# victorkich/ManyTor

Hardware: AMD Instinct MI355X
Metric: env-steps/sec (whole node), 1M parallel 4-DoF arms, random actions (higher is better)
Workload: dtype f32

## Files before the change

### manytor_amd/csrc/engine.hip

```cpp
#include <hip/hip_runtime.h>

#include <algorithm>
#include <cmath>
#include <cstdio>
#include <cstdlib>
#include <cstring>
#include <mutex>
#include <new>
#include <iterator>
#include <string>
#include <utility>
#include <vector>

#include "engine_internal.h"
#include "kernels.h"

using namespace mt;

namespace {
thread_local std::string g_last_error;
}

namespace mt {
int fail(mt_handle h, int code, const std::string& msg) {
// ... 148 lines not shown
  if (env_int("MT_RESET_SPLIT", &v)) {
    h->reset_split = v != 0;
    seen("MT_RESET_SPLIT");
  }
  h->graph_mode = -1;
  h->graph_max = P.graph_max;
  if (env_int("MT_GRAPH", &v)) {
    h->graph_mode = v != 0 ? 1 : 0;
    seen("MT_GRAPH");
  }
  h->flat_from = P.flat_from;
  if (env_int("MT_FLAT_FROM", &v)) {
    h->flat_from = std::max<long long>(0, v);
    seen("MT_FLAT_FROM");
  }
  h->blocks_per_cu_override = -1;
  if (env_int("MT_BLOCKS_PER_CU", &v)) {
    const int c = (int)std::max<long long>(0, std::min<long long>(8, v));
    h->blocks_per_cu_override = (c == 1 || c == 2) ? 3 : c;
    seen("MT_BLOCKS_PER_CU");
  }
  h->trig_steps = h->static_kind != 0;
  if (env_int("MT_TRIG_TABLE", &v)) {
    h->trig_steps = v != 0 && h->static_kind != 0;
    seen("MT_TRIG_TABLE");
  }

  h->chains = (n >= P.chains_min && n <= P.chains_max) ? 2 : 1;
  h->chains_forced = false;
  if (env_int("MT_CHAINS", &v)) {
    h->chains = (int)std::max<long long>(1, std::min<long long>(mt_engine::kMaxChains, v));
    h->chains_forced = true;
    seen("MT_CHAINS");
  }
  if (n < 2 * 256) h->chains = 1;
  h->lazy_chains = true;
  if (env_int("MT_LAZY_CHAINS", &v)) {
    h->lazy_chains = v != 0;
    seen("MT_LAZY_CHAINS");
  }

  h->multi_k = (n <= P.multi_step_max) ? P.multi_step_k : 1;
  if (env_int("MT_ROLLOUT_K", &v)) {
    h->multi_k = (int)std::max<long long>(1, std::min<long long>(64, v));
    seen("MT_ROLLOUT_K");
  }
  h->defer_reset = true;
  if (env_int("MT_DEFER_RESET", &v)) {
    h->defer_reset = v != 0;
    seen("MT_DEFER_RESET");
  }
  h->defer_reset_chained = P.fold_reset_into_chains;
  if (env_int("MT_DEFER_RESET_CHAINS", &v)) {
    h->defer_reset_chained = v != 0;
    seen("MT_DEFER_RESET_CHAINS");
  }
  h->gather_throttle = true;
  if (env_int("MT_GATHER_THROTTLE", &v)) {
    h->gather_throttle = v != 0;
    seen("MT_GATHER_THROTTLE");
  }
  h->snap_in_rollout = true;
  if (env_int("MT_ROLLOUT_SNAP", &v)) {
    h->snap_in_rollout = v != 0;
    seen("MT_ROLLOUT_SNAP");
  }
  h->rollout_early = true;
  if (env_int("MT_ROLLOUT_EARLY", &v)) {
    h->rollout_early = v != 0;
    seen("MT_ROLLOUT_EARLY");
  }

  h->tape_prefetch = false;
  if (env_int("MT_TAPE_PREFETCH", &v)) {
    h->tape_prefetch = v != 0;
    seen("MT_TAPE_PREFETCH");
  }
  h->tape_nt_loads = false;
  if (env_int("MT_TAPE_NT", &v)) {
    h->tape_nt_loads = v != 0;
    seen("MT_TAPE_NT");
  }

  if (h->custom_frames) h->lds_table = false;
  auto schedule_for = [&](int64_t envs, int64_t split4_max, int64_t split2_max, int64_t prefetch_other_max) {
    mt_engine::Schedule s;
    s.step_lanes = envs <= split4_max ? 4 : (envs <= split2_max ? 2 : 1);
    s.prefetch = h->static_kind == 1 || envs <= prefetch_other_max;
    s.rollout_lanes = envs <= P.fused_split4_max ? 4 : (envs <= P.fused_split2_max ? 2 : 1);
    if (forced_lanes) s.step_lanes = s.rollout_lanes = forced_lanes;
    if (forced_prefetch >= 0) s.prefetch = forced_prefetch != 0;
    if (h->custom_frames) s = mt_engine::Schedule{};
    return s;
  };
  h->sched[mt_engine::kBatch] = schedule_for(n, P.step_split4_max, P.step_split2_max, P.prefetch_other_max);
  h->sched[mt_engine::kChain] =
      h->chains > 1 ? schedule_for(chain_span(h, h->chains), P.chain_split4_max, P.chain_split2_max, P.chain_prefetch_other_max)
                    : h->sched[mt_engine::kBatch];
}

#define MT_DISPATCH_D(D_, FN, ...)   \
  switch (D_) {                      \
    case 2: FN<2>(__VA_ARGS__); break; \
    case 3: FN<3>(__VA_ARGS__); break; \
    case 4: FN<4>(__VA_ARGS__); break; \
    case 5: FN<5>(__VA_ARGS__); break; \
    case 6: FN<6>(__VA_ARGS__); break; \
    case 7: FN<7>(__VA_ARGS__); break; \
    case 8: FN<8>(__VA_ARGS__); break; \
    default: break;                  \
  }

struct StepVariant {
  int trig = 0;
  bool lds = false;
  int lanes = 1;
  int pf = 0;
  bool tt = false;
  bool flat = false;
  bool fresh = false;
  bool codes = false;
};
constexpr unsigned variant_key(const StepVariant& v) {
  return (unsigned)v.trig | (unsigned)v.lds << 3 | (unsigned)v.lanes << 4 | (unsigned)(v.pf != 0) << 7 | (unsigned)v.tt << 8 |
         (unsigned)v.flat << 9 | (unsigned)v.fresh << 10 | (unsigned)v.codes << 11;
}

#pragma clang diagnostic push
#pragma clang diagnostic ignored "-Wc++20-designator"
constexpr StepVariant kRuntimeVariants[] = {
    {.trig = 0}, {.trig = 1}, {.trig = 2}, {.trig = 3}, {.trig = 4}, {.trig = 5},
    {.lds = true},
    {.lanes = 2}, {.lanes = 4},
    {.pf = kPrefetch}, {.pf = kPrefetch, .flat = true},
};
constexpr StepVariant kFramesVariants[] = {{.trig = 0}, {.trig = 1}};
constexpr StepVariant kStaticVariants[] = {
    {.trig = 0}, {.trig = 1}, {.trig = 2}, {.trig = 3}, {.trig = 4}, {.trig = 5},
    {.lanes = 2}, {.lanes = 4},
    {.lanes = 2, .tt = true}, {.lanes = 4, .tt = true},
    {.pf = kPrefetch}, {.pf = kPrefetch, .flat = true},
    {.pf = 0, .tt = true}, {.pf = kPrefetch, .tt = true}, {.pf = kPrefetch, .tt = true, .flat = true},
    {.pf = kPrefetch, .tt = true, .codes = true}, {.pf = kPrefetch, .tt = true, .flat = true, .codes = true},
    {.pf = 0, .tt = true, .fresh = true}, {.pf = kPrefetch, .tt = true, .fresh = true},
    {.pf = kPrefetch, .tt = true, .flat = true, .fresh = true},
};
#pragma clang diagnostic pop

enum class TableKind { kRuntime = 0, kRef4 = 1, kDh7 = 2, kFrames = 3 };
struct StepPlan {
  TableKind table = TableKind::kRuntime;
  int D = 0;
  bool sample = false;
  StepVariant v;
  int blocks_per_cu = 0;
  size_t lds_bytes = 0;
  dim3 grid;
  bool exists = true;
};

StepPlan plan_step(const mt_engine* h, mt_engine::Scope scope, int64_t n, bool sample, bool codes, bool fresh = false) {
  const mt_engine::Schedule& s = h->sched[scope == mt_engine::kChain ? mt_engine::kChain : mt_engine::kBatch];
  const bool whole_rows = scope != mt_engine::kOneEnv;
  StepPlan p;
  p.table = h->custom_frames ? TableKind::kFrames : (TableKind)h->static_kind;
  p.D = h->D;
  p.sample = sample;
  p.grid = grid_for(n);
  StepVariant& v = p.v;
  if (fresh) {
    const size_t stage = (size_t)2 * h->K * kBlock * sizeof(float), fixed = kTrigEntries * sizeof(SinCos) + 512;
    p.exists = h->trig == 0 && h->trig_steps && s.step_lanes == 1 && !h->lds_table && !h->trace &&
               stage + fixed <= 65536;
    if (!p.exists) return p;
    p.sample = true;
    v.tt = v.fresh = true;
    v.pf = s.prefetch ? kPrefetch : 0;
    v.flat = v.pf && n >= h->flat_from;
    p.blocks_per_cu = v.pf ? step_blocks_per_cu(h, n) : 0;
    p.lds_bytes = std::max(stage, lds_pad_for_blocks(p.blocks_per_cu, fixed));
    return p;
  }
  if (p.table == TableKind::kFrames) {
    v.trig = h->trig == 1 ? 1 : 0;
    return p;
  }
  if (h->lds_table) {
    v.lds = true;
    return p;
  }
  if (h->trig != 0) {
    v.trig = h->trig;
    return p;
  }
  v.tt = sample && h->trig_steps && whole_rows;
  if (s.step_lanes > 1) {
    v.lanes = s.step_lanes;
    const int64_t per_block = kBlock / v.lanes;
    p.grid = dim3((unsigned)((n + per_block - 1) / per_block));
    return p;
  }
  v.pf = s.prefetch ? kPrefetch : 0;
  v.flat = v.pf && n >= h->flat_from;
  v.codes = v.pf && v.tt && codes;
  if (v.pf && v.tt) {
    p.blocks_per_cu = step_blocks_per_cu(h, n);
    p.lds_bytes = lds_pad_for_blocks(p.blocks_per_cu, kTrigEntries * sizeof(SinCos));
  }
  return p;
}

template <class Tbl, bool SAMPLE, const auto& ROWS, size_t I>
void launch_variant(const StepPlan& p, hipStream_t stream, const StepArgs& args) {
  constexpr StepVariant V = ROWS[I];
  if constexpr (V.lanes > 1)
    hipLaunchKernelGGL((step_split_kernel<Tbl, SAMPLE, V.lanes, V.tt>), p.grid, dim3(kBlock), p.lds_bytes, stream, args);
  else
    hipLaunchKernelGGL((step_kernel<Tbl, SAMPLE, V.trig, V.lds, V.pf, V.tt, V.flat, V.fresh, V.codes>), p.grid, dim3(kBlock),
                       p.lds_bytes, stream, args);
}
template <class Tbl, const auto& ROWS, size_t I>
bool launch_row(const StepPlan& p, hipStream_t stream, const StepArgs& args) {
  if (variant_key(p.v) != variant_key(ROWS[I])) return false;
  if (p.sample)
    launch_variant<Tbl, true, ROWS, I>(p, stream, args);
  else if constexpr (!ROWS[I].tt)
    launch_variant<Tbl, false, ROWS, I>(p, stream, args);
  else
    return false;
  return true;
}
template <class Tbl, const auto& ROWS, size_t... I>
bool launch_rows(const StepPlan& p, hipStream_t stream, const StepArgs& args, std::index_sequence<I...>) {
  return (launch_row<Tbl, ROWS, I>(p, stream, args) || ...);
}
template <class Tbl, const auto& ROWS>
bool launch_table(const StepPlan& p, hipStream_t stream, const StepArgs& args) {
  return launch_rows<Tbl, ROWS>(p, stream, args, std::make_index_sequence<std::size(ROWS)>{});
}
template <int D>
void launch_plan_d(const StepPlan& p, hipStream_t stream, const StepArgs& args, bool* launched) {
  *launched = p.table == TableKind::kFrames ? launch_table<RtTableF<D>, kFramesVariants>(p, stream, args)
                                            : launch_table<RtTable<D>, kRuntimeVariants>(p, stream, args);
}

void launch_plan(const StepPlan& p, hipStream_t stream, const StepArgs& args) {
  bool launched = false;
  if (p.table == TableKind::kRef4)
    launched = launch_table<Ref4Table, kStaticVariants>(p, stream, args);
  else if (p.table == TableKind::kDh7)
    launched = launch_table<Dh7Table, kStaticVariants>(p, stream, args);
  else
    MT_DISPATCH_D(p.D, launch_plan_d, p, stream, args, &launched);
  if (!launched) {
    std::fprintf(stderr, "manytor: no step kernel for table %d, D %d, sample %d, variant key 0x%x\n", (int)p.table, p.D,
                 (int)p.sample, variant_key(p.v));
    std::abort();
  }
}

template <int D>
void launch_trace_d(mt_handle h, const StepArgs& args, float* trace, bool sample) {
  if (sample)
    hipLaunchKernelGGL((trace_kernel<D, true>), grid_for(args.n), dim3(kBlock), 0, h->stream, args, trace);
  else
    hipLaunchKernelGGL((trace_kernel<D, false>), grid_for(args.n), dim3(kBlock), 0, h->stream, args, trace);
}

void launch_step(mt_handle h, mt_engine::Scope scope, const StepArgs& args, float* trace, bool sample) {
  if (trace) MT_DISPATCH_D(h->D, launch_trace_d, h, args, trace, sample);
  const StepPlan p = plan_step(h, scope, args.n, sample, h->codes_valid);
  launch_plan(p, h->stream, args);
  h->codes_valid = p.v.codes;
}

void launch_step(mt_handle h, bool sample) { launch_step(h, mt_engine::kBatch, h->args, h->trace, sample); }

bool launch_step_fresh(mt_handle h, mt_engine::Scope scope, const StepArgs& args) {
  const StepPlan p = plan_step(h, scope, args.n, true, false, true);
  if (!p.exists) return false;
  launch_plan(p, h->stream, args);
  h->codes_valid = p.v.codes;
  return true;
}

StepArgs args_for_range(mt_handle h, const StepArgs& base, int64_t off, int64_t cnt);
int check_launch(mt_handle h, const char* what);
int ensure_chains(mt_handle h, int chains) {
  if (!h->ev_fork) MT_HIP(h, hipEventCreateWithFlags(&h->ev_fork, event_flags(false)));
  for (int c = 1; c < chains; ++c) {
    if (!h->chain_streams[c]) MT_HIP(h, hipStreamCreateWithFlags(&h->chain_streams[c], hipStreamNonBlocking));
    if (!h->ev_join[c]) MT_HIP(h, hipEventCreateWithFlags(&h->ev_join[c], event_flags(false)));
  }
  return MT_OK;
}

void launch_chain(mt_handle h, const StepArgs& a0, uint32_t major0, int T, int chains, int c, bool sample = true) {
  const int64_t span = chain_span(h, chains), off = (int64_t)c * span;
  if (off >= h->n) return;
  StepArgs as = args_for_range(h, a0, off, std::min(span, h->n - off));
  for (int s = 0; s < T; ++s) {
    as.major = major0 + (uint32_t)s;
    launch_step(h, mt_engine::kChain, as, nullptr, sample);
  }
}

bool launch_chain_fresh(mt_handle h, const StepArgs& a0, uint32_t major, int chains, int c) {
  const int64_t span = chain_span(h, chains), off = (int64_t)c * span;
  if (off >= h->n) return true;
  StepArgs as = args_for_range(h, a0, off, std::min(span, h->n - off));
  as.major = major;
  return launch_step_fresh(h, mt_engine::kChain, as);
}

hipStream_t chain_stream(mt_handle h, int c) { return c == 0 ? h->stream : h->chain_streams[c]; }

int fork_chains(mt_handle h, int chains) {
  if (h->forked) return MT_OK;
  int rc = ensure_chains(h, chains);
  if (rc) return rc;
  const int64_t span = chain_span(h, chains);
  MT_HIP(h, hipEventRecord(h->ev_fork, h->stream));
  for (int c = 1; c < chains; ++c)
    if ((int64_t)c * span < h->n) MT_HIP(h, hipStreamWaitEvent(h->chain_streams[c], h->ev_fork, 0));
  h->forked = true;
  return MT_OK;
}

int settle_chains(mt_handle h) { return (h->lazy_chains && h->stream == h->own_stream) ? MT_OK : join_chains(h); }

// ... 432 lines not shown
    }
    if (h->ev_join[c]) (void)hipEventDestroy(h->ev_join[c]);
    if (h->ev1c[c]) (void)hipEventDestroy(h->ev1c[c]);
  }
  if (h->ev_fork) (void)hipEventDestroy(h->ev_fork);
  if (h->graph_step0) (void)hipFree(h->graph_step0);
  if (h->staging) (void)hipFree(h->staging);
  if (h->pinned) (void)hipHostFree(h->pinned);
  if (h->arena) (void)hipFree(h->arena);
  if (h->ev0) (void)hipEventDestroy(h->ev0);
  if (h->ev1) (void)hipEventDestroy(h->ev1);
  for (hipEvent_t e : h->lap_events) (void)hipEventDestroy(e);
  if (h->own_stream) (void)hipStreamDestroy(h->own_stream);
  delete h;
  return MT_OK;
}

static StepPlan batch_plan(const mt_engine* h) { return plan_step(h, mt_engine::kBatch, h->n, true, false); }
static StepPlan chain_plan(const mt_engine* h) { return plan_step(h, mt_engine::kChain, chain_span(h, h->chains), true, false); }
static std::string table_name(const mt_engine* h) {
  const char* tbl = h->static_kind == 1 ? "Ref4Table" : (h->static_kind == 2 ? "Dh7Table" : nullptr);
  return tbl ? tbl : (h->custom_frames ? "RtTableF<" : "RtTable<") + std::to_string(h->D) + ">";
}
static int multi_step_lanes(const mt_engine* h) {
  return h->sched[(h->chains > 1 && h->chains_forced) ? mt_engine::kChain : mt_engine::kBatch].rollout_lanes;
}

const char* mt_step_kernel_name(mt_handle h) {
  if (!h) return "";
  const std::string table = table_name(h);
  const StepVariant v = batch_plan(h).v;
  if (v.lanes > 1)
    h->kernel_name = "step_split_kernel<" + table + ", L=" + std::to_string(v.lanes) + (v.tt ? ", tt=1>" : ">");
  else
    h->kernel_name = "step_kernel<" + table + ", trig=" + std::to_string(h->trig) + ", lds=" + (v.lds ? "true" : "false") +
                     ", pf=" + std::to_string(v.pf) + (v.tt ? ", tt=1" : "") + (v.flat ? ", flat=1>" : ">");
  const bool multi_one_chain = h->multi_k > 1 && fusable(h) && !h->chains_forced;
  if (h->chains > 1 && !multi_one_chain) {
    const StepPlan c = chain_plan(h);
    h->kernel_name += " [mt_rollout: " + std::to_string(h->chains) + " chains of " + std::to_string(chain_span(h, h->chains)) +
                      " envs, " + (c.v.lanes > 1 ? "L=" + std::to_string(c.v.lanes)
                                                 : "pf=" + std::to_string(c.v.pf) + (c.v.flat ? ", flat=1" : "")) +
                      (c.blocks_per_cu > 0 ? ", " + std::to_string(c.blocks_per_cu) + " blocks/CU" : std::string()) + "]";
  }
  if (h->multi_k > 1 && fusable(h)) {
    const int sp = multi_step_lanes(h);
    h->kernel_name += " [mt_rollout: " + std::to_string(h->multi_k) + " steps per launch, " +
                      (sp > 1 ? "rollout_split_kernel L=" + std::to_string(sp) : std::string("rollout_kernel")) + "]";
  }
  return h->kernel_name.c_str();
}

const char* mt_describe_dispatch(mt_handle h) {
  if (!h) return "";
  const DispatchPolicy& P = kPolicy;
  auto num = [](long long v) { return std::to_string(v); };
  auto b = [](bool v) { return std::string(v ? "true" : "false"); };
  const int64_t span = chain_span(h, h->chains);
  const std::string table = table_name(h);
  const StepPlan sb = batch_plan(h), sc = chain_plan(h);
  const bool multi = h->multi_k > 1 && fusable(h);
  const bool graph = h->graph_mode > 0 || (h->graph_mode < 0 && h->n <= h->graph_max);
  std::string caps = "[";
  for (const BlockCap& c : P.block_caps) caps += std::string(caps.size() > 1 ? "," : "") + "[" + num(c.from) + "," + num(c.below) + "," + num(c.blocks) + "]";
  caps += "]";
  std::string& d = h->describe;
  d = "{\"n_envs\":" + num(h->n) + ",\"ld\":" + num(h->ld) + ",\"dof\":" + num(h->D) + ",\"targets\":" + num(h->K) +
      ",\"table\":\"" + table + "\",\"trig\":" + num(h->trig) + ",\"lds_table\":" + b(h->lds_table) + ",\"custom_frames\":" + b(h->custom_frames) +
      ",\"step\":{\"lanes_per_env\":" + num(sb.v.lanes) + ",\"prefetch\":" + b(sb.v.pf != 0) +
      ",\"trig_table\":" + b(sb.v.tt) + ",\"flat\":" + b(sb.v.flat) + "}" +
      ",\"chains\":{\"count\":" + num(h->chains) + ",\"span\":" + num(h->chains > 1 ? span : h->n) + ",\"lazy\":" + b(h->lazy_chains) +
      ",\"lanes_per_env\":" + num(sc.v.lanes) + ",\"prefetch\":" + b(sc.v.pf != 0) + ",\"flat\":" + b(sc.v.flat) +
      ",\"blocks_per_cu\":" + num(h->chains > 1 ? sc.blocks_per_cu : 0) + "}" +
      ",\"rollout\":{\"form\":\"" + (multi ? "multi_step" : (h->chains > 1 ? "chained_steps" : (graph ? "graph_replay" : "launch_per_step"))) +
      "\",\"steps_per_launch\":" + num(multi ? h->multi_k : 1) + ",\"graph\":" + b(!multi && graph) +
      ",\"lanes_per_env\":" + num(multi ? multi_step_lanes(h) : (h->chains > 1 ? sc : sb).v.lanes) +
      ",\"chains\":" + num(multi && !h->chains_forced ? 1 : h->chains) +
      ",\"absorbs_reset\":" + b(h->defer_reset && (multi || chained_rollout_absorbs_reset(h))) + ",\"writes_snapshot\":" + b(h->snap_in_rollout && (multi || (h->chains > 1 && !graph && !h->trace))) + "}" +
      ",\"fused\":{\"usable\":" + b(fusable(h)) + ",\"lanes_per_env\":" + num(h->sched[mt_engine::kBatch].rollout_lanes) + "}" +
      ",\"tape\":{\"usable\":" + b(fusable(h)) + ",\"lanes_per_env\":1,\"chains\":1,\"prefetch\":" + b(tape_prefetches(h)) +
      ",\"nt_loads\":" + b(h->tape_nt_loads) + "}" +
      ",\"shoot\":{\"usable\":" + b(fusable(h)) + ",\"envs_per_block\":" + num(kShootEnvs) + ",\"waves_per_block\":" + num(kShootWaves) + "}" +
      ",\"reset\":{\"lanes_per_env\":" + num(h->reset_split ? 4 : 1) + "}" +
      ",\"overrides\":\"" + h->overrides + "\"" +
      ",\"policy\":{\"step_split4_max\":" + num(P.step_split4_max) + ",\"step_split2_max\":" + num(P.step_split2_max) +
      ",\"prefetch_other_max\":" + num(P.prefetch_other_max) + ",\"fused_split4_max\":" + num(P.fused_split4_max) +
      ",\"fused_split2_max\":" + num(P.fused_split2_max) + ",\"reset_split_max\":" + num(P.reset_split_max) +
      ",\"graph_max\":" + num(P.graph_max) + ",\"chains_min\":" + num(P.chains_min) + ",\"chains_max\":" + num(P.chains_max) +
      ",\"chain_split4_max\":" + num(P.chain_split4_max) + ",\"chain_split2_max\":" + num(P.chain_split2_max) +
      ",\"chain_prefetch_other_max\":" + num(P.chain_prefetch_other_max) + ",\"flat_from\":" + num(P.flat_from) +
      ",\"block_caps\":" + caps + ",\"multi_step_max\":" + num(P.multi_step_max) + ",\"multi_step_k\":" + num(P.multi_step_k) +
      ",\"max_recurrence_rotations\":" + num(P.max_recurrence_rotations) + ",\"ld_pad_above\":" + num(P.ld_pad_above) +
      ",\"ld_pad_floats\":" + num(P.ld_pad_floats) + "}" +
      ",\"arena_bytes\":" + num((long long)h->arena_bytes) + "}";
  return d.c_str();
}

int mt_set_stream(mt_handle h, void* hip_stream) {
  MT_REQUIRE(nullptr, h != nullptr, "handle is NULL");
  MT_ENTER(h);
  MT_HIP(h, hipStreamSynchronize(h->stream));
  h->stream = (hipStream_t)hip_stream;
  return MT_OK;
}

int mt_use_own_stream(mt_handle h) {
  MT_REQUIRE(nullptr, h != nullptr, "handle is NULL");
  MT_ENTER(h);
  MT_HIP(h, hipStreamSynchronize(h->stream));
  h->stream = h->own_stream;
  return MT_OK;
}

int mt_sync(mt_handle h) {
  MT_REQUIRE(nullptr, h != nullptr, "handle is NULL");
  MT_ENTER(h);
  MT_HIP(h, hipStreamSynchronize(h->stream));
  if (h->gather_pending) {
    MT_HIP(h, hipStreamSynchronize(h->side_stream));
    MT_HIP(h, hipEventElapsedTime(&h->last_gather_ms, h->ev_g0, h->ev_g1));
    h->gather_pending = false;
    h->snap_free_known[0] = h->snap_free_known[1] = true;
  }
  return MT_OK;
}

int mt_reset(mt_handle h, const float* points, int layout, int is_device) {
  MT_REQUIRE(nullptr, h != nullptr, "handle is NULL");
  MT_REQUIRE(h, points != nullptr, "points is NULL (use mt_reset_random for device-drawn targets)");
  MT_REQUIRE(h, layout == MT_ENV_MAJOR || layout == MT_SOA, "bad layout");
  if (!is_device && layout == MT_ENV_MAJOR) {
    const int64_t bad = first_unusable(points, h->n * 3 * h->K, kMaxFiniteBits);
    if (bad >= 0) return fail(h, MT_ERR_INVALID_ARG, "mt_reset: points element " + std::to_string(bad) + " is NaN or infinite");
  }
  if (!is_device && layout == MT_SOA)
    for (int r = 0; r < 3 * h->K; ++r) {
      const int64_t bad = first_unusable(points + (int64_t)r * h->ld, h->n, kMaxFiniteBits);
      if (bad >= 0)
        return fail(h, MT_ERR_INVALID_ARG, "mt_reset: points row " + std::to_string(r) + " element " + std::to_string(bad) + " is NaN or infinite");
    }
  MT_ENTER(h);
  const int rows = 3 * h->K;
  if (layout == MT_SOA) {
    const size_t bytes = (size_t)rows * h->ld * 4;
    MT_HIP(h, hipMemcpyAsync(h->args.points, points, bytes, is_device ? hipMemcpyDeviceToDevice : hipMemcpyHostToDevice,
                             h->stream));
  } else {
    const size_t bytes = (size_t)rows * h->n * 4;
    const float* src = points;
    if (!is_device) {
      int rc = ensure_staging(h, bytes);
      if (rc) return rc;
      MT_HIP(h, hipMemcpyAsync(h->staging, points, bytes, hipMemcpyHostToDevice, h->stream));
      src = (const float*)h->staging;
    }
    hipLaunchKernelGGL((env_major_to_soa<float>), grid_for(h->n), dim3(kBlock), 0, h->stream, src, rows, h->n,
                       h->args.points, h->ld);
    int rc = check_launch(h, "env_major_to_soa");
    if (rc) return rc;
  }
  {
    int rcg = order_behind_inplace_gather(h, h->stream);
    if (rcg) return rcg;
  }
  h->args.major = 0;
  h->args.episode0 = 0;
// ... 1259 lines not shown
```

### manytor_amd/csrc/engine_internal.h

```cpp
#pragma once
#include <hip/hip_runtime.h>

#include <cstdlib>
#include <string>
#include <vector>

#include "step_args.h"

struct mt_comm;

struct mt_engine {
  static constexpr int kMaxChains = 4;
  mt_config cfg{};
  int64_t n = 0, ld = 0;
  int D = 0, K = 0;
  hipStream_t own_stream = nullptr;
  hipStream_t stream = nullptr;
  hipEvent_t ev0 = nullptr, ev1 = nullptr;
  hipEvent_t ev1c[kMaxChains] = {nullptr, nullptr, nullptr, nullptr};
  int timer_ends = 0;
  bool timer_with_gather = false;
  struct LapRec {
    uint32_t begin, n_begin, end0, n_end;
  };
  std::vector<hipEvent_t> lap_events;
  size_t lap_events_used = 0;
  std::vector<LapRec> lap_recs;
  bool lap_open = false;
  void* arena = nullptr;
  size_t arena_bytes = 0;
  void* staging = nullptr;
  size_t staging_bytes = 0;
  void* pinned = nullptr;
  size_t pinned_bytes = 0;
  mt::StepArgs args{};
  float* trace = nullptr;
  unsigned long long* spare_bits = nullptr;
  bool is_reset = false;
  int trig = 0;
  bool lds_table = false;
  bool custom_frames = false;
  struct Schedule {
    int step_lanes = 1;
    bool prefetch = false;
    int rollout_lanes = 1;
  };
  enum Scope { kBatch = 0, kChain = 1, kOneEnv = 2 };
  Schedule sched[2];
  int blocks_per_cu_override = -1;
  int64_t flat_from = 393216;
  bool goals_exposed = false;
  bool codes_valid = false;
  bool points_exposed = false;
  bool trig_steps = false;
  int static_kind = 0;
  mt_comm* comm = nullptr;
  hipStream_t side_stream = nullptr;
  hipEvent_t ev_snap = nullptr, ev_g0 = nullptr, ev_g1 = nullptr;
  float* snap = nullptr;
  hipEvent_t ev_gdone[2] = {nullptr, nullptr};
  bool snap_free_known[2] = {true, true};
  int snap_next = 0;
  bool gather_throttle = true;
  float* snap_row(int p) const { return snap + (size_t)p * (size_t)n; }
  void* reduce_scratch = nullptr;
  size_t reduce_scratch_bytes = 0;
  bool reset_split = false;
  struct RolloutGraph {
    int T;
    int chains;
    mt::StepArgs args;
    hipGraphExec_t exec[kMaxChains];
  };
  std::vector<RolloutGraph> graphs;
  std::vector<int> graph_seen;
  uint32_t* graph_step0 = nullptr;
  int graph_mode = -1;
  int64_t graph_max = 131072;
  int chains = 1;
  bool chains_forced = false;
  int multi_k = 1;
  bool rollout_early = true;
  bool defer_reset_chained = false;
  bool defer_reset = true;
  bool reset_pending = false;
  uint64_t pend_seed = 0;
  uint32_t pend_episode = 0;
  bool snap_in_rollout = true;
  bool snap_valid = false;
  bool tape_prefetch = false;
  bool tape_nt_loads = false;
  std::string overrides;
  std::string describe;
  hipStream_t chain_streams[kMaxChains] = {nullptr, nullptr, nullptr, nullptr};
  hipEvent_t ev_fork = nullptr, ev_join[kMaxChains] = {nullptr, nullptr, nullptr, nullptr};
  bool forked = false;
  bool lazy_chains = true;
  bool gather_pending = false;
  bool gather_inplace = false;
  float last_gather_ms = 0.f;
  std::string err;
  std::string kernel_name;
};

namespace mt {

inline unsigned event_flags(bool timing) {
  static const bool fenced = [] {
    const char* e = std::getenv("MT_EVENT_FENCE");
    return e && *e && std::atoi(e) != 0;
  }();
  return (timing ? 0u : (unsigned)hipEventDisableTiming) | (fenced ? 0u : (unsigned)hipEventDisableSystemFence);
}

int fail(mt_handle h, int code, const std::string& msg);

class DeviceGuard {
 public:
  explicit DeviceGuard(int device) {
    if (hipGetDevice(&prev_) != hipSuccess) prev_ = -1;
    err_ = (prev_ == device) ? hipSuccess : hipSetDevice(device);
    changed_ = (err_ == hipSuccess && prev_ != device);
  }
  ~DeviceGuard() {
    if (changed_ && prev_ >= 0) (void)hipSetDevice(prev_);
  }
  hipError_t error() const { return err_; }

 private:
  int prev_ = -1;
  hipError_t err_ = hipSuccess;
  bool changed_ = false;
};

inline dim3 grid_for(int64_t n) { return dim3((unsigned)((n + kBlock - 1) / kBlock)); }

inline bool snapshot_trusted(mt_engine* h) {
  if (h->stream != h->own_stream) return false;
  hipStreamCaptureStatus st = hipStreamCaptureStatusNone;
  if (hipStreamIsCapturing(h->stream, &st) != hipSuccess) {
    (void)hipGetLastError();
    return false;
  }
  return st == hipStreamCaptureStatusNone;
}

int join_chains(mt_handle h);
int flush_pending_reset(mt_handle h);

}

#define MT_HIP(h, call)                                                                            \
  do {                                                                                             \
    hipError_t e__ = (call);                                                                       \
    if (e__ != hipSuccess)                                                                         \
      return mt::fail(h, MT_ERR_HIP, std::string(#call) + ": " + hipGetErrorString(e__));          \
  } while (0)

#define MT_REQUIRE(h, cond, msg)                              \
  do {                                                        \
    if (!(cond)) return mt::fail(h, MT_ERR_INVALID_ARG, msg); \
  } while (0)

#define MT_ON_DEVICE(h, device)                                                                          \
  mt::DeviceGuard mt_guard__(device);                                                                    \
  if (mt_guard__.error() != hipSuccess)                                                                  \
  return mt::fail(h, MT_ERR_HIP, std::string("hipSetDevice: ") + hipGetErrorString(mt_guard__.error()))

#define MT_ENTER(h)                              \
  MT_ON_DEVICE(h, (h)->cfg.device);              \
  do {                                           \
    (h)->snap_valid = false;                     \
    if ((h)->forked) {                           \
      int rcj__ = mt::join_chains(h);            \
// ... 20 lines not shown
```

### manytor_amd/csrc/kernels.h

```cpp
#pragma once
#include <hip/hip_runtime.h>
#include <stdint.h>

#include "mt_math.h"
#include "philox.h"
#include "step_args.h"

namespace mt {

#ifndef MT_NT_STORES
#define MT_NT_STORES 1
#endif
template <typename T>
using global_ptr = __attribute__((address_space(1))) T*;

__device__ __forceinline__ global_ptr<char> uniform_row(const void* row) {
  const uint64_t v = reinterpret_cast<uint64_t>(row);
  const uint32_t lo = __builtin_amdgcn_readfirstlane((uint32_t)v);
  const uint32_t hi = __builtin_amdgcn_readfirstlane((uint32_t)(v >> 32));
  return (global_ptr<char>)(((uint64_t)hi << 32) | lo);
}
#ifndef MT_PLAIN_LANE_OFFSET
#define MT_PLAIN_LANE_OFFSET 0
#endif
template <bool RENEW>
struct LaneOffset {
  uint32_t v;
};
template <bool RENEW>
__device__ __forceinline__ uint32_t lane_offset(LaneOffset<RENEW>& o) {
#if !MT_PLAIN_LANE_OFFSET
  if (RENEW) asm volatile("" : "+v"(o.v));
#endif
  return o.v;
}
#ifndef MT_BUFFER_ROWS
#define MT_BUFFER_ROWS 0
#endif
#if MT_BUFFER_ROWS
constexpr int kRsrcWord3 = 0x00020000;
constexpr int kAuxNt = 2;
__device__ __forceinline__ __amdgpu_buffer_rsrc_t row_rsrc(const void* row) {
  return __builtin_amdgcn_make_buffer_rsrc((void*)uniform_row(row), 0, -1, kRsrcWord3);
}
template <typename T, bool R>
__device__ __forceinline__ T ldr(const T* row, LaneOffset<R>& o) {
  static_assert(sizeof(T) == 4 || sizeof(T) == 1, "rows hold 32-bit words or bytes");
  if constexpr (sizeof(T) == 4)
    return __builtin_bit_cast(T, __builtin_amdgcn_raw_buffer_load_b32(row_rsrc(row), (int)o.v, 0, 0));
  else
    return __builtin_bit_cast(T, __builtin_amdgcn_raw_buffer_load_b8(row_rsrc(row), (int)o.v, 0, 0));
}
template <typename T, bool R>
__device__ __forceinline__ void str(T* row, LaneOffset<R>& o, T v) {
  static_assert(sizeof(T) == 4 || sizeof(T) == 1, "rows hold 32-bit words or bytes");
  if constexpr (sizeof(T) == 4)
    __builtin_amdgcn_raw_buffer_store_b32(__builtin_bit_cast(uint32_t, v), row_rsrc(row), (int)o.v, 0, 0);
  else
    __builtin_amdgcn_raw_buffer_store_b8(__builtin_bit_cast(uint8_t, v), row_rsrc(row), (int)o.v, 0, 0);
}
template <typename T, bool R>
__device__ __forceinline__ void str_stream(T* row, LaneOffset<R>& o, T v) {
  static_assert(sizeof(T) == 4 || sizeof(T) == 1, "rows hold 32-bit words or bytes");
  constexpr int aux = MT_NT_STORES ? kAuxNt : 0;
  if constexpr (sizeof(T) == 4)
    __builtin_amdgcn_raw_buffer_store_b32(__builtin_bit_cast(uint32_t, v), row_rsrc(row), (int)o.v, 0, aux);
  else
    __builtin_amdgcn_raw_buffer_store_b8(__builtin_bit_cast(uint8_t, v), row_rsrc(row), (int)o.v, 0, aux);
}
#else
template <typename T, bool R>
__device__ __forceinline__ T ldr(const T* row, LaneOffset<R>& o) {
  return *(global_ptr<const T>)(uniform_row(row) + lane_offset(o));
}
template <typename T, bool R>
__device__ __forceinline__ void str(T* row, LaneOffset<R>& o, T v) {
  *(global_ptr<T>)(uniform_row(row) + lane_offset(o)) = v;
}
template <typename T, bool R>
__device__ __forceinline__ void str_stream(T* row, LaneOffset<R>& o, T v) {
  global_ptr<T> p = (global_ptr<T>)(uniform_row(row) + lane_offset(o));
#if MT_NT_STORES
  __builtin_nontemporal_store(v, p);
#else
  *p = v;
// ... 506 lines not shown
      for (int j = 1; j < JN; ++j) {
        const float pose = __builtin_fmaf(fk, st[j], gq[j]);
        if (TRIG == 2)
          sincos_deg_hw(pose, sF[j], cF[j]);
        else
          sincos_deg(pose, sF[j], cF[j]);
      }
      chain_z<Tbl>(sF, cF, t, zo, ze);
      zmin = fminf(zmin, fminf(zo, ze));
    }
  }
  return zmin;
}

template <class Tbl, bool TABLE>
__device__ __forceinline__ bool wide_route(const float (&g)[Tbl::D], const float (&act)[Tbl::D], bool prev_whole) {
  float reach = 0.f;
  if (!prev_whole) {
#pragma unroll
    for (int j = 0; j < Tbl::D; ++j) reach = fmaxf(reach, __builtin_fabsf(g[j]));
  }
  if (!TABLE) {
#pragma unroll
    for (int j = 0; j < Tbl::D; ++j) reach = fmaxf(reach, __builtin_fabsf(act[j]));
  }
  return wide_angle(reach);
}

template <class Tbl, bool CACHED>
__device__ __forceinline__ float route_kinematics_wide(const Tbl& t, int S, const float (&g)[Tbl::D],
                                                       const float (&act)[Tbl::D], float (&el)[3], float (&e)[3],
                                                       PoseCache<Tbl::D>* cache) {
  constexpr int D = Tbl::D;
  constexpr int JN = ZJoints<Tbl>::value;
  float s[D], c[D];
#pragma unroll
  for (int j = 0; j < D; ++j) {
    s[j] = 0.f;
    c[j] = 1.f;
  }
  float zmin = 0.f;
  const double inv = 1.0 / (double)(S - 1);
  for (int k = 0; k < S - 1; ++k) {
    const double frac = (double)k * inv;
#pragma unroll
    for (int j = 1; j < JN; ++j) {
      float gj = g[j], aj = act[j];
      asm volatile("" : "+v"(gj), "+v"(aj));
      sincos_deg_route(gj, aj, frac, t.off(j), s[j], c[j]);
    }
    float zo, ze;
    chain_z<Tbl>(s, c, t, zo, ze);
    zmin = (k == 0) ? fminf(zo, ze) : fminf(zmin, fminf(zo, ze));
  }
  float p[D][3];
#pragma unroll
  for (int j = 0; j < D; ++j) sincos_deg_off(act[j], t.off(j), s[j], c[j]);
  chain_all<Tbl>(s, c, t, p);
  pick_frames<Tbl>(t, p, el, e);
  if (CACHED) {
#pragma unroll
    for (int j = 1; j < JN; ++j) {
      cache->s[j] = s[j];
      cache->c[j] = c[j];
    }
    cache->zmin = fminf(el[2], e[2]);
  }
  zmin = fminf(zmin, fminf(el[2], e[2]));
  return zmin;
}

template <class Tbl, int TRIG, bool CACHED = false, bool TABLE = false>
__device__ __forceinline__ float route_kinematics(const Tbl& t, int S, float inv_sm1, const float (&g)[Tbl::D],
                                                  const float (&act)[Tbl::D], float (&el)[3], float (&e)[3],
                                                  PoseCache<Tbl::D>* cache = nullptr, bool cache_valid = false,
                                                  const SinCos* trig = nullptr, bool prev_whole = false) {
  if constexpr (TRIG <= 2) {
    if (__builtin_expect(__any(wide_route<Tbl, TABLE>(g, act, prev_whole)), 0))
      return route_kinematics_wide<Tbl, CACHED>(t, S, g, act, el, e, cache);
  }
  return route_kinematics_narrow<Tbl, TRIG, CACHED, TABLE>(t, S, inv_sm1, g, act, el, e, cache, cache_valid, trig, prev_whole);
}

__device__ __forceinline__ void record_finished(const StepArgs& a, uint32_t i, uint32_t episode, float ret) {
  LaneOffset<true> o4{i * 4u};
  str(a.last_return, o4, ret);
  if (a.ring_slots)
    a.ring[(int64_t)((episode - a.episode0) % a.ring_slots) * a.ld + i] = ret;
}

#ifdef MT_STAMPS
#define MT_STAMP(a, i, slot)                                                                 \
  do {                                                                                       \
    __builtin_amdgcn_sched_barrier(0);                                                       \
    unsigned long long t__;                                                                  \
    asm volatile("s_memtime %0\n\ts_waitcnt lgkmcnt(0)" : "=s"(t__)::"memory");              \
    __builtin_amdgcn_sched_barrier(0);                                                       \
    if ((a).stamps && (threadIdx.x & 63) == 0) (a).stamps[(size_t)((i) >> 6) * 8 + (slot)] = t__; \
  } while (0)
#else
#define MT_STAMP(a, i, slot) \
  do {                       \
  } while (0)
#endif

__device__ __forceinline__ bool unusable_angle(float v) { return (__float_as_uint(v) & 0x7FFFFFFFu) > 0x47000000u; }

template <class Tbl, int TRIG>
constexpr int step_min_waves() { return (TRIG == 0 && Tbl::D >= 6 && Tbl::D <= 7) ? 8 : 1; }

constexpr int kPrefetch = 8;

__device__ __forceinline__ void draw_targets_wave(uint64_t seed, uint64_t env0, uint32_t episode, bool need, int K, float radius,
                                                  float* col0, uint8_t* slots);

template <class Tbl, bool SAMPLE, int TRIG, bool LDS, int PF = 0, bool TT = false, bool FLAT = false, bool FRESH = false,
          bool CODES = false>
__global__ __launch_bounds__(kBlock, (PF ? 1 : step_min_waves<Tbl, TRIG>())) void step_kernel(const StepArgs a) {
  constexpr int D = Tbl::D;
  static_assert(!TT || (SAMPLE && TRIG == 0 && !LDS && ActionTrigTable<Tbl>::value), "the table serves sampled actions of a static table");
  static_assert(!FRESH || TT, "the reset prologue exists for the sampled-action kernels of the static tables");
  static_assert(!CODES || (PF && TT && !FRESH), "codes are read by the prefetch kernels of the static tables");
  extern __shared__ float fresh_stage[];
  __shared__ uint8_t fresh_slots[FRESH ? kBlock / 64 : 1][64];
  __shared__ DhConst sh;
  __shared__ __attribute__((aligned(16))) SinCos trig_lds[TT ? kTrigEntries : 1];
  float4 trig_v;
  if (TT) trig_v = trig_table_load(a.trig_table);
  if (LDS) {
    const float* src = reinterpret_cast<const float*>(&a.dh);
    float* dst = reinterpret_cast<float*>(&sh);
    if (threadIdx.x < sizeof(DhConst) / sizeof(float)) dst[threadIdx.x] = src[threadIdx.x];
    __syncthreads();
  }
  const Tbl t = TableMaker<Tbl>::make(LDS ? sh : a.dh);

  const uint32_t i = blockIdx.x * kBlock + threadIdx.x;
  LaneOffset<!FLAT> o4{i * 4u}, o1{i};
  if (!TT && i >= a.n) return;
  const int64_t ld = a.ld;
  const uint32_t step_no = SAMPLE ? step_index(a) : 0u;

  constexpr bool kLean = D >= 6;
  MT_STAMP(a, i, 0);
  float g[D], act[D];
#pragma unroll
  for (int j = 0; j < D; ++j) g[j] = FRESH ? 0.f : ldr(a.goals + j * ld, o4);
  float tx[PF ? PF : 1][3];
  uint32_t tc[CODES ? PF : 1][2];
  if constexpr (FRESH) {
    const bool mine = i < a.n;
    const uint32_t lane = threadIdx.x & 63u;
    if (mine) {
      str(a.last_return, o4, ldr(a.total_reward, o4));
      str(a.episodes, o4, a.reset_episode);
    }
    draw_targets_wave(((uint64_t)a.reset_seed_hi << 32) | a.reset_seed_lo, (uint64_t)(a.env_base + (i - lane)), a.reset_episode, mine,
                      a.K, a.radius, fresh_stage + (threadIdx.x - lane), fresh_slots[threadIdx.x >> 6]);
    if (mine) {
      const float* col = fresh_stage + threadIdx.x;
#pragma unroll
      for (int k = 0; k < (PF ? PF : 0); ++k)
        if (k < a.K) {
          decode_target(staged_code(col + 2 * k * kBlock, kBlock), a.radius, tx[k][0], tx[k][1], tx[k][2]);
#pragma unroll
          for (int q = 0; q < 3; ++q) str(a.points + (int64_t)(3 * k + q) * ld, o4, tx[k][q]);
        }
      for (int k = PF; k < a.K; ++k) {
        float x, y, z;
        decode_target(staged_code(col + 2 * k * kBlock, kBlock), a.radius, x, y, z);
        const int64_t r = 3 * k;
        str(a.points + r * ld, o4, x);
        str(a.points + (r + 1) * ld, o4, y);
        str(a.points + (r + 2) * ld, o4, z);
      }
    }
  } else if (PF) {
#pragma unroll
    for (int k = 0; k < PF; ++k)
      if (k < a.K) {
        if constexpr (CODES) {
          const uint32_t* crow = a.codes + (int64_t)(2 * k) * ld;
          tc[k][0] = ldr(crow, o4);
          tc[k][1] = ldr(crow + ld, o4);
        } else {
          const float* row = a.points + (int64_t)(3 * k) * ld;
#pragma unroll
          for (int q = 0; q < 3; ++q) tx[k][q] = ldr(row + q * ld, o4);
        }
      }
  }
  uint32_t am = 0;
  float total_in = 0.f;
  if (FRESH) {
    am = (a.K >= 32) ? 0xFFFFFFFFu : ((1u << a.K) - 1u);
  } else if (!kLean || PF) {
    am = ldr(a.alive, o4);
    total_in = ldr(a.total_reward, o4);
  }
  if (SAMPLE) {
    draw_action<D>(((uint64_t)a.seed_hi << 32) | a.seed_lo, (uint64_t)(a.env_base + i), step_no, act);
  } else {
    bool bad = false;
#pragma unroll
    for (int j = 0; j < D; ++j) {
      act[j] = ldr(a.actions + j * ld, o4);
      bad |= unusable_angle(act[j]);
    }
    if (bad) {
#pragma unroll
      for (int j = 0; j < D; ++j) act[j] = g[j];
      atomicAdd(a.bad_actions, 1u);
    }
  }
  MT_STAMP(a, i, 1);
  if (TT) {
    trig_table_commit(trig_lds, trig_v);
    if (i >= a.n) return;
  }
  if (kLean) {
#pragma unroll
    for (int j = 0; j < D; ++j) str(a.goals + j * ld, o4, act[j]);
  }

  float el[3], e[3];
  const float zmin = route_kinematics<Tbl, TRIG, false, TT>(t, a.S, a.inv_sm1, g, act, el, e, nullptr, false, trig_lds,
                                                            (a.flags & kFlagWholeGoals) != 0);
  const bool ground = zmin < 0.f;
  if (a.zmin) str_stream(a.zmin, o4, zmin);
  if (kLean && !PF && !FRESH) {
    am = ldr(a.alive, o4);
    total_in = ldr(a.total_reward, o4);
  }
  MT_STAMP(a, i, 2);

  uint32_t nam = am;
  if (PF) {
#pragma unroll
    for (int k = 0; k < PF; ++k)
      if (k < a.K) {
        if constexpr (CODES) decode_target(TargetCode{tc[k][0], tc[k][1]}, a.radius, tx[k][0], tx[k][1], tx[k][2]);
        step_target<false, CODES>(a, ld, o4, k, am, nam, el, e, tx[k][0], tx[k][1], tx[k][2]);
      }
  }
  for (int k = PF; k < a.K; ++k) {
    if (TRIG == 5) {
      float dist, r, th;
      const float x = (float)(i & 63) + (float)k, y = 3.0f + (float)k, z = 5.0f + g[0];
      observe_target(el, x, y, z, dist, r, th);
      if (within_box(e, x, y, z, a.tol)) nam &= ~(1u << k);
      if (dist + r + th == -12345.0f) (a.obs + (int64_t)(3 * k) * ld)[i] = dist;
      continue;
    }
    if constexpr (CODES) {
      const uint32_t* crow = a.codes + (int64_t)(2 * k) * ld;
      float x, y, z;
      decode_target(TargetCode{ldr(crow, o4), ldr(crow + ld, o4)}, a.radius, x, y, z);
      step_target<false, true>(a, ld, o4, k, am, nam, el, e, x, y, z);
      continue;
    }
    const float* row = a.points + (int64_t)(3 * k) * ld;
    {
      const float x = ldr(row, o4), y = ldr(row + ld, o4), z = ldr(row + 2 * ld, o4);
      step_target<TRIG == 4>(a, ld, o4, k, am, nam, el, e, x, y, z);
    }
  }

  MT_STAMP(a, i, 3);
  const int32_t rew = ground ? -1 : ((nam != am) ? 1 : 0);
  bool done = (nam == 0u);
  if (a.flags & MT_FLAG_TERMINATE_ON_GROUND) done |= ground;

  if (!kLean) {
#pragma unroll
    for (int j = 0; j < D; ++j) str(a.goals + j * ld, o4, act[j]);
  }
#pragma unroll
  for (int q = 0; q < 3; ++q) str_stream(a.ee + q * ld, o4, e[q]);
  str(a.alive, o4, nam);
  str_stream(a.reward, o4, rew);
  str(a.total_reward, o4, total_in + (float)rew);
  if (a.snap) str(a.snap, o4, total_in + (float)rew);
  str_stream(a.done, o1, (uint8_t)(done ? 1 : 0));
  const unsigned long long bits = __ballot(done);
  if ((threadIdx.x & 63) == 0) a.done_bits[i >> 6] = bits;
  MT_STAMP(a, i, 4);
#ifdef MT_STAMPS
  asm volatile("s_waitcnt vmcnt(0)" ::: "memory");
  MT_STAMP(a, i, 5);
#endif
}

template <class Tbl, int L, bool CACHED, bool TABLE>
__device__ __forceinline__ float route_kinematics_split_narrow(const Tbl& t, int S, float inv_sm1, const float (&g)[Tbl::D],
                                                               const float (&act)[Tbl::D], bool backward, float (&el)[3],
                                                               float (&e)[3], PoseCache<Tbl::D>* cache, bool cache_valid,
                                                               const SinCos* trig, bool prev_whole) {
  constexpr int D = Tbl::D;
  constexpr int JN = ZJoints<Tbl>::value;
  constexpr int EPW = 64 / L;
  const bool use_cache = CACHED && __all(cache_valid);
  float st[D];
#pragma unroll
  for (int j = 0; j < D; ++j) st[j] = (act[j] - g[j]) * inv_sm1;
  float sA[D], cA[D], p3[D][3];
  action_sincos<Tbl, TABLE>(t, act, sA, cA, trig);
  chain_all<Tbl>(sA, cA, t, p3);
  pick_frames<Tbl>(t, p3, el, e);
  float sF[D], cF[D];
#pragma unroll
// ... 1364 lines not shown
```

Before: 31.05 billion.

## Compact undecided ground-collision routes into a block-wide LDS queue split across lanes

Adds a block-cooperative ground test, on by default for D<=5 static or runtime tables. After the endpoint check, lanes whose route is still undecided are queued in LDS. Each queued route is then split into forward and backward halves, which two lanes evaluate in parallel. This is meant to cut wave divergence, where a few lanes step through the full route interpolation while the rest sit idle. In exchange the kernel uses more LDS, which may lower occupancy, adds two block barriers, and keeps out-of-range threads alive until the barrier.

Measured after the change: 32.22 billion, median of 6. +3.8%, better.

```diff
diff --git a/manytor_amd/csrc/engine.hip b/manytor_amd/csrc/engine.hip
--- a/manytor_amd/csrc/engine.hip
+++ b/manytor_amd/csrc/engine.hip
@@ -254,6 +254,12 @@
     seen("MT_TAPE_NT");
   }
 
+  h->ground_compact = true;
+  if (env_int("MT_GROUND_COMPACT", &v)) {
+    h->ground_compact = v != 0;
+    seen("MT_GROUND_COMPACT");
+  }
+
   if (h->custom_frames) h->lds_table = false;
   auto schedule_for = [&](int64_t envs, int64_t split4_max, int64_t split2_max, int64_t prefetch_other_max) {
     mt_engine::Schedule s;
@@ -292,10 +298,11 @@
   bool flat = false;
   bool fresh = false;
   bool codes = false;
+  bool gc = false;
 };
 constexpr unsigned variant_key(const StepVariant& v) {
   return (unsigned)v.trig | (unsigned)v.lds << 3 | (unsigned)v.lanes << 4 | (unsigned)(v.pf != 0) << 7 | (unsigned)v.tt << 8 |
-         (unsigned)v.flat << 9 | (unsigned)v.fresh << 10 | (unsigned)v.codes << 11;
+         (unsigned)v.flat << 9 | (unsigned)v.fresh << 10 | (unsigned)v.codes << 11 | (unsigned)v.gc << 12;
 }
 
 #pragma clang diagnostic push
@@ -305,6 +312,7 @@
     {.lds = true},
     {.lanes = 2}, {.lanes = 4},
     {.pf = kPrefetch}, {.pf = kPrefetch, .flat = true},
+    {.gc = true}, {.pf = kPrefetch, .gc = true}, {.pf = kPrefetch, .flat = true, .gc = true},
 };
 constexpr StepVariant kFramesVariants[] = {{.trig = 0}, {.trig = 1}};
 constexpr StepVariant kStaticVariants[] = {
@@ -316,6 +324,9 @@
     {.pf = kPrefetch, .tt = true, .codes = true}, {.pf = kPrefetch, .tt = true, .flat = true, .codes = true},
     {.pf = 0, .tt = true, .fresh = true}, {.pf = kPrefetch, .tt = true, .fresh = true},
     {.pf = kPrefetch, .tt = true, .flat = true, .fresh = true},
+    {.gc = true}, {.pf = kPrefetch, .gc = true}, {.pf = kPrefetch, .flat = true, .gc = true},
+    {.pf = 0, .tt = true, .gc = true}, {.pf = kPrefetch, .tt = true, .gc = true}, {.pf = kPrefetch, .tt = true, .flat = true, .gc = true},
+    {.pf = kPrefetch, .tt = true, .codes = true, .gc = true}, {.pf = kPrefetch, .tt = true, .flat = true, .codes = true, .gc = true},
 };
 #pragma clang diagnostic pop
 
@@ -330,6 +341,20 @@
   dim3 grid;
   bool exists = true;
 };
+
+static bool ground_compacts(const mt_engine* h, bool whole_rows) {
+  return h->ground_compact && whole_rows && h->trig == 0 && !h->lds_table && !h->custom_frames &&
+         !(h->cfg.flags & MT_FLAG_DEBUG_ZMIN) && h->D <= 5;
+}
+template <int D>
+static void ground_queue_bytes_d(size_t* out) { *out = sizeof(GroundQueue<RtTable<D>>); }
+static size_t ground_queue_bytes(const mt_engine* h) {
+  if (h->static_kind == 1) return sizeof(GroundQueue<Ref4Table>);
+  if (h->static_kind == 2) return sizeof(GroundQueue<Dh7Table>);
+  size_t bytes = 0;
+  MT_DISPATCH_D(h->D, ground_queue_bytes_d, &bytes);
+  return bytes;
+}
 
 StepPlan plan_step(const mt_engine* h, mt_engine::Scope scope, int64_t n, bool sample, bool codes, bool fresh = false) {
   const mt_engine::Schedule& s = h->sched[scope == mt_engine::kChain ? mt_engine::kChain : mt_engine::kBatch];
@@ -375,9 +400,10 @@
   v.pf = s.prefetch ? kPrefetch : 0;
   v.flat = v.pf && n >= h->flat_from;
   v.codes = v.pf && v.tt && codes;
+  v.gc = ground_compacts(h, whole_rows);
   if (v.pf && v.tt) {
     p.blocks_per_cu = step_blocks_per_cu(h, n);
-    p.lds_bytes = lds_pad_for_blocks(p.blocks_per_cu, kTrigEntries * sizeof(SinCos));
+    p.lds_bytes = lds_pad_for_blocks(p.blocks_per_cu, kTrigEntries * sizeof(SinCos) + (v.gc ? ground_queue_bytes(h) : 0));
   }
   return p;
 }
@@ -388,13 +414,15 @@
   if constexpr (V.lanes > 1)
     hipLaunchKernelGGL((step_split_kernel<Tbl, SAMPLE, V.lanes, V.tt>), p.grid, dim3(kBlock), p.lds_bytes, stream, args);
   else
-    hipLaunchKernelGGL((step_kernel<Tbl, SAMPLE, V.trig, V.lds, V.pf, V.tt, V.flat, V.fresh, V.codes>), p.grid, dim3(kBlock),
+    hipLaunchKernelGGL((step_kernel<Tbl, SAMPLE, V.trig, V.lds, V.pf, V.tt, V.flat, V.fresh, V.codes, V.gc>), p.grid, dim3(kBlock),
                        p.lds_bytes, stream, args);
 }
 template <class Tbl, const auto& ROWS, size_t I>
 bool launch_row(const StepPlan& p, hipStream_t stream, const StepArgs& args) {
   if (variant_key(p.v) != variant_key(ROWS[I])) return false;
-  if (p.sample)
+  if constexpr (ROWS[I].gc && Tbl::D >= 6)
+    return false;
+  else if (p.sample)
     launch_variant<Tbl, true, ROWS, I>(p, stream, args);
   else if constexpr (!ROWS[I].tt)
     launch_variant<Tbl, false, ROWS, I>(p, stream, args);
@@ -418,6 +446,10 @@
 
 void launch_plan(const StepPlan& p, hipStream_t stream, const StepArgs& args) {
   bool launched = false;
+  if (p.v.gc && (int64_t)p.grid.x * kBlock > args.ld) {
+    std::fprintf(stderr, "manytor: a ground-compacting step launch of %u blocks over rows of %lld\n", p.grid.x, (long long)args.ld);
+    std::abort();
+  }
   if (p.table == TableKind::kRef4)
     launched = launch_table<Ref4Table, kStaticVariants>(p, stream, args);
   else if (p.table == TableKind::kDh7)
@@ -1016,6 +1048,7 @@
       ",\"nt_loads\":" + b(h->tape_nt_loads) + "}" +
       ",\"shoot\":{\"usable\":" + b(fusable(h)) + ",\"envs_per_block\":" + num(kShootEnvs) + ",\"waves_per_block\":" + num(kShootWaves) + "}" +
       ",\"reset\":{\"lanes_per_env\":" + num(h->reset_split ? 4 : 1) + "}" +
+      ",\"ground_compact\":{\"enabled\":" + b(h->ground_compact) + ",\"step\":" + b(sb.v.gc) + ",\"chains\":" + b(sc.v.gc) + "}" +
       ",\"overrides\":\"" + h->overrides + "\"" +
       ",\"policy\":{\"step_split4_max\":" + num(P.step_split4_max) + ",\"step_split2_max\":" + num(P.step_split2_max) +
       ",\"prefetch_other_max\":" + num(P.prefetch_other_max) + ",\"fused_split4_max\":" + num(P.fused_split4_max) +
diff --git a/manytor_amd/csrc/engine_internal.h b/manytor_amd/csrc/engine_internal.h
--- a/manytor_amd/csrc/engine_internal.h
+++ b/manytor_amd/csrc/engine_internal.h
@@ -90,6 +90,7 @@
   bool snap_valid = false;
   bool tape_prefetch = false;
   bool tape_nt_loads = false;
+  bool ground_compact = true;
   std::string overrides;
   std::string describe;
   hipStream_t chain_streams[kMaxChains] = {nullptr, nullptr, nullptr, nullptr};
diff --git a/manytor_amd/csrc/kernels.h b/manytor_amd/csrc/kernels.h
--- a/manytor_amd/csrc/kernels.h
+++ b/manytor_amd/csrc/kernels.h
@@ -1,6 +1,8 @@
 #pragma once
 #include <hip/hip_runtime.h>
 #include <stdint.h>
+
+#include <type_traits>
 
 #include "mt_math.h"
 #include "philox.h"
@@ -673,6 +675,134 @@
   return route_kinematics_narrow<Tbl, TRIG, CACHED, TABLE>(t, S, inv_sm1, g, act, el, e, cache, cache_valid, trig, prev_whole);
 }
 
+template <class Tbl>
+struct GroundQueue {
+  static constexpr int kJoints = ZJoints<Tbl>::value - 1;
+  static constexpr int kFields = 6 * kJoints;
+  static constexpr int kCap = (14336 / (4 * kFields) >= kBlock / 2) ? kBlock / 2 : (14336 / (4 * kFields)) / 32 * 32;
+  static_assert(kCap >= 32 && 2 * kCap <= kBlock, "one half route per lane");
+  uint32_t count;
+  float zres[2 * kCap];
+  float field[kFields][kCap];
+};
+
+template <class Tbl>
+__device__ __forceinline__ float half_route_zmin(const Tbl& t, float (&s)[Tbl::D], float (&c)[Tbl::D], const float (&sd)[Tbl::D],
+                                                 const float (&cd)[Tbl::D], int n_half, int mine) {
+  constexpr int D = Tbl::D;
+  constexpr int JN = ZJoints<Tbl>::value;
+  float zm = 3.0e38f, zo, ze;
+#pragma unroll 2
+  for (int it = 1; it <= n_half; ++it) {
+    rotate_pose<D, JN, +1>(s, c, sd, cd);
+    chain_z<Tbl>(s, c, t, zo, ze);
+    if (it <= mine) zm = fminf(zm, fminf(zo, ze));
+  }
+  return zm;
+}
+
+struct NoGroundQueue {
+  uint32_t count;
+};
+__device__ __forceinline__ void ground_queue_reset(uint32_t* count) {
+  if (threadIdx.x == 0) *count = 0u;
+}
+
+template <class Tbl, bool TABLE>
+__device__ __forceinline__ float route_kinematics_block(const Tbl& t, int S, float inv_sm1, const float (&g)[Tbl::D],
+                                                        const float (&act)[Tbl::D], float (&el)[3], float (&e)[3],
+                                                        const SinCos* trig, bool prev_whole, bool live, GroundQueue<Tbl>& q) {
+  constexpr int D = Tbl::D;
+  constexpr int JN = ZJoints<Tbl>::value;
+  constexpr int kCap = GroundQueue<Tbl>::kCap;
+  const int nf = (S - 1) / 2;
+  const int nb = S - 2 - nf;
+  float zmin;
+  bool undecided = false;
+  float sF[D], cF[D], sA[D], cA[D], sd[D], cd[D];
+  if (__builtin_expect(__any(live && wide_route<Tbl, TABLE>(g, act, prev_whole)), 0)) {
+    zmin = route_kinematics_wide<Tbl, false>(t, S, g, act, el, e, nullptr);
+  } else {
+    float st[D];
+#pragma unroll
+    for (int j = 0; j < D; ++j) st[j] = (act[j] - g[j]) * inv_sm1;
+    float p[D][3], zo, ze;
+    action_sincos<Tbl, TABLE>(t, act, sA, cA, trig);
+    chain_all<Tbl>(sA, cA, t, p);
+    pick_frames<Tbl>(t, p, el, e);
+    zmin = fminf(el[2], e[2]);
+#pragma unroll
+    for (int j = 0; j < D; ++j) {
+      sF[j] = 0.f;
+      cF[j] = 1.f;
+    }
+    prev_pose_sincos<Tbl, TABLE>(t, g, sF, cF, trig, prev_whole);
+    chain_z<Tbl>(sF, cF, t, zo, ze);
+    zmin = fminf(zmin, fminf(zo, ze));
+    sincos_increment<D, JN>(st, sd, cd);
+    sA[0] = 0.f;
+    cA[0] = 1.f;
+    undecided = live && !(zmin < 0.f);
+  }
+
+  const unsigned long long um = __ballot(undecided);
+  uint32_t slot = kCap;
+  if (um != 0ull) {
+    uint32_t base = 0u;
+    if ((threadIdx.x & 63u) == 0u) base = atomicAdd(&q.count, (uint32_t)__popcll(um));
+    base = (uint32_t)__builtin_amdgcn_readfirstlane((int)base);
+    slot = base + __builtin_amdgcn_mbcnt_hi((uint32_t)(um >> 32), __builtin_amdgcn_mbcnt_lo((uint32_t)um, 0u));
+  }
+  const bool queued = undecided && slot < (uint32_t)kCap;
+  if (queued) {
+#pragma unroll
+    for (int j = 1; j < JN; ++j) {
+      float(*f)[kCap] = q.field + 6 * (j - 1);
+      f[0][slot] = sF[j];
+      f[1][slot] = cF[j];
+      f[2][slot] = sA[j];
+      f[3][slot] = cA[j];
+      f[4][slot] = sd[j];
+      f[5][slot] = cd[j];
+    }
+  }
+  if (undecided && !queued) {
+    zmin = fminf(zmin, half_route_zmin<Tbl>(t, sF, cF, sd, cd, nf, nf));
+#pragma unroll
+    for (int j = 1; j < JN; ++j) sd[j] = -sd[j];
+    zmin = fminf(zmin, half_route_zmin<Tbl>(t, sA, cA, sd, cd, nf, nb));
+  }
+  __syncthreads();
+
+  const uint32_t routes = q.count < (uint32_t)kCap ? q.count : (uint32_t)kCap;
+  const uint32_t w = (threadIdx.x + 64u * (blockIdx.x & 3u)) & (uint32_t)(kBlock - 1);
+  if (w < 2u * routes) {
+    const uint32_t r = w >> 1;
+    const bool backward = (w & 1u) != 0u;
+    float sW[D], cW[D], sdW[D], cdW[D];
+#pragma unroll
+    for (int j = 0; j < D; ++j) {
+      sW[j] = 0.f;
+      cW[j] = 1.f;
+      sdW[j] = 0.f;
+      cdW[j] = 1.f;
+    }
+#pragma unroll
+    for (int j = 1; j < JN; ++j) {
+      const float(*f)[kCap] = q.field + 6 * (j - 1);
+      sW[j] = backward ? f[2][r] : f[0][r];
+      cW[j] = backward ? f[3][r] : f[1][r];
+      const float sdj = f[4][r];
+      sdW[j] = backward ? -sdj : sdj;
+      cdW[j] = f[5][r];
+    }
+    q.zres[w] = half_route_zmin<Tbl>(t, sW, cW, sdW, cdW, nf, backward ? nb : nf);
+  }
+  __syncthreads();
+  if (queued) zmin = fminf(zmin, fminf(q.zres[2u * slot], q.zres[2u * slot + 1u]));
+  return zmin;
+}
+
 __device__ __forceinline__ void record_finished(const StepArgs& a, uint32_t i, uint32_t episode, float ret) {
   LaneOffset<true> o4{i * 4u};
   str(a.last_return, o4, ret);
@@ -706,9 +836,10 @@
                                                   float* col0, uint8_t* slots);
 
 template <class Tbl, bool SAMPLE, int TRIG, bool LDS, int PF = 0, bool TT = false, bool FLAT = false, bool FRESH = false,
-          bool CODES = false>
+          bool CODES = false, bool GC = false>
 __global__ __launch_bounds__(kBlock, (PF ? 1 : step_min_waves<Tbl, TRIG>())) void step_kernel(const StepArgs a) {
   constexpr int D = Tbl::D;
+  static_assert(!GC || (TRIG == 0 && !LDS && !FRESH), "the block-cooperative ground test serves the recurrence");
   static_assert(!TT || (SAMPLE && TRIG == 0 && !LDS && ActionTrigTable<Tbl>::value), "the table serves sampled actions of a static table");
   static_assert(!FRESH || TT, "the reset prologue exists for the sampled-action kernels of the static tables");
   static_assert(!CODES || (PF && TT && !FRESH), "codes are read by the prefetch kernels of the static tables");
@@ -716,8 +847,13 @@
   __shared__ uint8_t fresh_slots[FRESH ? kBlock / 64 : 1][64];
   __shared__ DhConst sh;
   __shared__ __attribute__((aligned(16))) SinCos trig_lds[TT ? kTrigEntries : 1];
+  __shared__ std::conditional_t<GC, GroundQueue<Tbl>, NoGroundQueue> ground_q;
   float4 trig_v;
   if (TT) trig_v = trig_table_load(a.trig_table);
+  if constexpr (GC) {
+    ground_queue_reset(&ground_q.count);
+    if (!TT) __syncthreads();
+  }
   if (LDS) {
     const float* src = reinterpret_cast<const float*>(&a.dh);
     float* dst = reinterpret_cast<float*>(&sh);
@@ -728,7 +864,8 @@
 
   const uint32_t i = blockIdx.x * kBlock + threadIdx.x;
   LaneOffset<!FLAT> o4{i * 4u}, o1{i};
-  if (!TT && i >= a.n) return;
+  const bool live = i < a.n;
+  if (!TT && !GC && !live) return;
   const int64_t ld = a.ld;
   const uint32_t step_no = SAMPLE ? step_index(a) : 0u;
 
@@ -801,22 +938,36 @@
     if (bad) {
 #pragma unroll
       for (int j = 0; j < D; ++j) act[j] = g[j];
-      atomicAdd(a.bad_actions, 1u);
+      if (!GC || live) atomicAdd(a.bad_actions, 1u);
+    }
+  }
+  if constexpr (GC) {
+#pragma unroll
+    for (int j = 0; j < D; ++j) {
+      g[j] = live ? g[j] : 0.f;
+      if (!SAMPLE) act[j] = live ? act[j] : 0.f;
     }
   }
   MT_STAMP(a, i, 1);
   if (TT) {
     trig_table_commit(trig_lds, trig_v);
-    if (i >= a.n) return;
-  }
-  if (kLean) {
+    if (!GC && !live) return;
+  }
+  if (kLean && (!GC || live)) {
 #pragma unroll
     for (int j = 0; j < D; ++j) str(a.goals + j * ld, o4, act[j]);
   }
 
   float el[3], e[3];
-  const float zmin = route_kinematics<Tbl, TRIG, false, TT>(t, a.S, a.inv_sm1, g, act, el, e, nullptr, false, trig_lds,
-                                                            (a.flags & kFlagWholeGoals) != 0);
+  float zmin;
+  if constexpr (GC) {
+    zmin = route_kinematics_block<Tbl, TT>(t, a.S, a.inv_sm1, g, act, el, e, trig_lds, (a.flags & kFlagWholeGoals) != 0, live,
+                                           ground_q);
+    if (!live) return;
+  } else {
+    zmin = route_kinematics<Tbl, TRIG, false, TT>(t, a.S, a.inv_sm1, g, act, el, e, nullptr, false, trig_lds,
+                                                  (a.flags & kFlagWholeGoals) != 0);
+  }
   const bool ground = zmin < 0.f;
   if (a.zmin) str_stream(a.zmin, o4, zmin);
   if (kLean && !PF && !FRESH) {
```
